# HNUicda/CoIVO

Hardware: AMD Instinct MI355X
Metric: training frame-pairs/sec at 320x256 (higher is better)
Workload: dtype bf16

## Files before the change

### coivo_amd/csrc/wgrad.hip

```cpp
#define COLVO_ACC_CONSTRAINT "+a"
#include "conv_common.h"

namespace colvo {
namespace {

template <typename T, int MT>
constexpr int dy_pitch() {
#ifdef COLVO_WGRAD_OLD_LAYOUT
    return 16 * MT * TT<T>::ES + 16;
#else
    if (TT<T>::ES == 4) return 16 * MT * 4 + 16;
    return MT == 1 ? 32 : MT == 2 ? 96 : 160;
#endif
}

template <typename T, int MT, int NG, bool TAIL, int KS = 1>
__global__ __launch_bounds__(NT * KS) void k_wgrad3x3(const WgradK a) {
    constexpr int G = TT<T>::G, ES = TT<T>::ES;
    constexpr int CK = NG * G;
    constexpr int NCOL = 9 * CK;
    constexpr int NFR = (NCOL + 15) / 16;
    constexpr int FPW = (NFR + 3) / 4;
    constexpr int PIXP = TAIL ? pitch_bytes_s2(NG * 16) : pitch_bytes(NG * 16);
    constexpr int DYP = dy_pitch<T, MT>();
    extern __shared__ __attribute__((aligned(16))) char smem[];
#ifdef COLVO_WTRACE
    long long wt_start = (long long)clock64(), wt_first = 0, wt_store = 0, wt_compute = 0, wt_b1 = 0, wt_b2 = 0, wt_loop_end = 0, wt_flush = 0;
    long long wt_issue = 0, wt_mfma = 0, wt_m0 = 0, wt_m1 = 0;
    long long wt_wall0 = (long long)wall_clock64();
#define WT_STAMP(x) x = (long long)clock64()
#else
#define WT_STAMP(x) do {} while (0)
#endif
    const int tid = threadIdx.x & (NT - 1), lane = tid & 63, wave = tid >> 6;
    const int team = (KS > 1) ? __builtin_amdgcn_readfirstlane(threadIdx.x / NT) : 0;
    const int l15 = lane & 15, kg = lane >> 4;
    const int lid = __builtin_amdgcn_readfirstlane(xcd_remap(blockIdx.x, gridDim.x, a.xcd));
    const int per_split = gridDim.x / a.nsplit;
    const int bsplit = lid / per_split, brem = lid - bsplit * per_split;
    const int bchunk = brem / a.cot, bco = brem - bchunk * a.cot;
    const int co0 = bco * 16 * MT;
    const int chunks0 = a.g.C[0] / CK;
    const int s = (bchunk < chunks0) ? 0 : 1;
    const int c0 = (s == 0 ? bchunk : bchunk - chunks0) * CK;
    const int wc0 = (s == 0 ? 0 : a.g.C[0]) + c0;
    const int S = a.g.stride;
    const int PH = (a.toh - 1) * S + 3, PW = (a.tow - 1) * S + 3;
    const int npix = a.toh * a.tow;
    const int PWL = a.pwl;
    const int stage = (BM * DYP + PH * PWL * PIXP + 15) & ~15;
    char* sDY = smem + team * stage;
    char* sX = sDY + BM * DYP;

    int boff[FPW];
    int ocol[FPW];
#pragma unroll
    for (int fi = 0; fi < FPW; ++fi) {
        const int f = wave + 4 * fi;
        const int ncol_addr = 16 * f + ((ES == 2) ? 4 * (lane & 3) : l15);
        int tap = min(ncol_addr / CK, 8);
        const int c = ncol_addr - (ncol_addr / CK) * CK;
        boff[fi] = ((tap / 3) * PWL + (tap % 3)) * PIXP + c * ES;
        const int ncol = 16 * f + l15;
        ocol[fi] = (f < NFR && ncol < NCOL) ? ((ncol / CK) * a.Ctot + (ncol % CK)) : -1;
    }

    f32x4 acc[MT][FPW];
#pragma unroll
    for (int mi = 0; mi < MT; ++mi)
#pragma unroll
        for (int fi = 0; fi < FPW; ++fi) acc[mi][fi] = f32x4{0.f, 0.f, 0.f, 0.f};
    float dbacc = 0.0f;

    const int t_begin = bsplit * a.tiles_per_split;
    const int t_end = min(a.ntiles, t_begin + a.tiles_per_split);
    const int tiles_per_img = a.tiles_x * a.tiles_y;

    constexpr int DGR = 16 * MT / G;
    constexpr int DIT = (BM * DGR + NT - 1) / NT;
    constexpr int PPF = TAIL ? 9 : 3;
    const int ptotal = PH * PW * NG;
    u32x4 dyv[DIT], pv[PPF];

    struct TileC { int b, ty, tx; };
    auto tile_next = [&](TileC& c) {
        if (++c.tx == a.tiles_x) { c.tx = 0; if (++c.ty == a.tiles_y) { c.ty = 0; ++c.b; } }
    };
    TileC cur;
    {
        const int t = __builtin_amdgcn_readfirstlane(t_begin + team);
        cur.b = t / tiles_per_img;
        const int tr_ = t - cur.b * tiles_per_img;
        cur.ty = tr_ / a.tiles_x; cur.tx = tr_ - cur.ty * a.tiles_x;
    }
    const long long dy_bytes = (long long)a.B * a.Ho * a.Wo * a.Cout * ES;
    const long long x_bytes = (long long)a.B * a.g.Hs[s] * a.g.Ws[s] * a.g.C[s] * ES;
    const __amdgpu_buffer_rsrc_t rdy = __builtin_amdgcn_make_buffer_rsrc((void*)a.dy, 0, (int)(dy_bytes < 0x7fffffffLL ? dy_bytes : 0x7fffffffLL), 0x00020000);
    const __amdgpu_buffer_rsrc_t rx = __builtin_amdgcn_make_buffer_rsrc((void*)a.g.src[s], 0, (int)(x_bytes < 0x7fffffffLL ? x_bytes : 0x7fffffffLL), 0x00020000);
    const int Hs = a.g.Hs[s], Ws = a.g.Ws[s], Cs = a.g.C[s];
    const int sh = (a.g.mode[s] != MODE_DIRECT) ? 1 : 0;

    int dy_off[DIT], dy_yx[DIT], dy_lds[DIT];
#pragma unroll
    for (int it = 0; it < DIT; ++it) {
        const int i = it * NT + tid;
        const int pp_ = i / DGR, gch = i - pp_ * DGR;
        const int oy = mdiv(pp_, a.m_tow), ox = pp_ - oy * a.tow;
        const bool ok = (BM * DGR % NT == 0 || i < BM * DGR) && (pp_ < npix) && (co0 + gch * G < a.Cout);
        dy_off[it] = ok ? ((oy * a.Wo + ox) * a.Cout + co0 + gch * G) * ES : OOB_OFF;
        dy_yx[it] = (oy << 16) | ox;
        dy_lds[it] = pp_ * DYP + gch * 16;
    }
    int p_yx[PPF], p_cg[PPF], p_lds[PPF];
#pragma unroll
    for (int it = 0; it < PPF; ++it) {
        const int i = it * NT + tid;
        const int pix = i / NG;
        p_cg[it] = i - pix * NG;
        const int py = mdiv(pix, a.m_pw), px = pix - py * PW;
        p_yx[it] = (i < ptotal) ? ((py << 16) | px) : (0x7fff << 16);
        p_lds[it] = (py * PWL + px) * PIXP + p_cg[it] * 16;
    }
    auto load_dy = [&](const TileC& c, bool live) {
        const int oy0 = c.ty * a.toh, ox0 = c.tx * a.tow;
        const int base = live ? ((c.b * a.Ho + oy0) * a.Wo + ox0) * a.Cout * ES : 0;
        const int remy = live ? a.Ho - oy0 : 0, remx = a.Wo - ox0;
        if (remy >= a.toh && remx >= a.tow) {
#pragma unroll
            for (int it = 0; it < DIT; ++it) dyv[it] = bld16(rdy, dy_off[it], base);
        } else {
#pragma unroll
            for (int it = 0; it < DIT; ++it) {
                const bool ok = ((dy_yx[it] >> 16) < remy) && ((dy_yx[it] & 0xffff) < remx);
                dyv[it] = bld16(rdy, ok ? dy_off[it] : OOB_OFF, base);
            }
        }
    };
    auto store_dy = [&]() {
#pragma unroll
        for (int it = 0; it < DIT; ++it)
            if (BM * DGR % NT == 0 || it * NT + tid < BM * DGR) st16(sDY + dy_lds[it], dyv[it]);
    };
    auto patch_voff = [&](const TileC& c, int yx, int cg) -> int {
        const int vy = c.ty * a.toh * S - 1 + (yx >> 16), vx = c.tx * a.tow * S - 1 + (yx & 0xffff);
        const bool inb = ((unsigned)vy < (unsigned)a.g.Hi) && ((unsigned)vx < (unsigned)a.g.Wi);
        return inb ? (((vy >> sh) * Ws + (vx >> sh)) * Cs + c0 + cg * G) * ES : OOB_OFF;
    };
    auto load_p = [&](const TileC& c, bool live) {
        const int base = live ? c.b * Hs * Ws * Cs * ES : 0;
        const int dead = live ? 0 : OOB_OFF;
#pragma unroll
        for (int it = 0; it < PPF; ++it) pv[it] = bld16(rx, patch_voff(c, p_yx[it], p_cg[it]) | dead, base);
    };
    auto store_p = [&](const TileC& c, bool live) {
#pragma unroll
        for (int it = 0; it < PPF; ++it) {
            const int i = it * NT + tid;
            if (i < ptotal) st16(sX + p_lds[it], pv[it]);
        }
        const int base = live ? c.b * Hs * Ws * Cs * ES : 0;
        const int dead = live ? 0 : OOB_OFF;
        if constexpr (TAIL)
        for (int g0 = PPF * NT; g0 < ptotal; g0 += 3 * NT) {
            u32x4 tt[3];
            int tl[3];
#pragma unroll
            for (int u = 0; u < 3; ++u) {
                const int i = g0 + u * NT + tid;
                const int pix = i / NG, cg = i - pix * NG;
                const int py = mdiv(pix, a.m_pw), px = pix - py * PW;
                tt[u] = bld16(rx, ((i < ptotal) ? patch_voff(c, (py << 16) | px, cg) : OOB_OFF) | dead, base);
                tl[u] = (py * PWL + px) * PIXP + cg * 16;
            }
#pragma unroll
            for (int u = 0; u < 3; ++u)
                if (g0 + u * NT + tid < ptotal) st16(sX + tl[u], tt[u]);
        }
    };
    constexpr int NPH = NT / (16 * MT);
    const int db_co = tid % (16 * MT), db_ph = tid / (16 * MT);

    if (t_begin < t_end) { const bool live = t_begin + team < t_end; load_dy(cur, live); load_p(cur, live); }
    for (int t = t_begin; t < t_end; t += KS) {
        __syncthreads();
#ifdef COLVO_WTRACE
        WT_STAMP(wt_b1);
        if (t == t_begin) wt_first = wt_b1; else wt_compute += wt_b1 - wt_b2;
#endif
        store_dy();
        store_p(cur, t + team < t_end);
        __syncthreads();
#ifdef COLVO_WTRACE
        WT_STAMP(wt_b2);
        wt_store += wt_b2 - wt_b1;
#endif
#pragma unroll
        for (int q = 0; q < KS; ++q) tile_next(cur);
        if (t + KS < t_end) { const bool live = t + KS + team < t_end; load_dy(cur, live); load_p(cur, live); }

        if (bchunk == 0 && a.db) {
            float s0 = 0.0f, s1 = 0.0f;
#pragma unroll 4
            for (int p = db_ph; p < BM; p += 2 * NPH) {
                if constexpr (ES == 2) {
                    s0 += bf2f(*reinterpret_cast<const uint16_t*>(sDY + p * DYP + db_co * 2));
                    s1 += bf2f(*reinterpret_cast<const uint16_t*>(sDY + (p + NPH) * DYP + db_co * 2));
                } else {
                    s0 += *reinterpret_cast<const float*>(sDY + p * DYP + db_co * 4);
                    s1 += *reinterpret_cast<const float*>(sDY + (p + NPH) * DYP + db_co * 4);
                }
            }
            dbacc += s0 + s1;
        }

#ifdef COLVO_WTRACE
        WT_STAMP(wt_m0);
        wt_issue += wt_m0 - wt_b2;
#endif
        if constexpr (ES == 2) {
            const int q = l15 >> 2, pp = lane & 3;
            auto read_step = [&](int ks, s16x8 (&af)[MT], s16x8 (&bfv)[FPW]) {
                int xo[2], yo[2];
#pragma unroll
                for (int h = 0; h < 2; ++h) {
#ifdef COLVO_WGRAD_OLD_LAYOUT
                    int p = 32 * ks + 8 * kg + q + 4 * h;
#else
                    int p = 32 * ks + 16 * (kg >> 1) + 8 * h + 4 * (kg & 1) + q;
#endif
                    yo[h] = p * DYP;
                    if (p >= npix) p = 0;
                    const int oy = mdiv(p, a.m_tow), ox = p - oy * a.tow;
                    xo[h] = ((oy * S) * PWL + ox * S) * PIXP;
                }
#pragma unroll
                for (int mi = 0; mi < MT; ++mi) {
                    const s16x4 lo = __builtin_amdgcn_ds_read_tr16_b64_v4i16(
                        (__attribute__((address_space(3))) s16x4*)(sDY + yo[0] + (16 * mi + 4 * pp) * 2));
                    const s16x4 hi = __builtin_amdgcn_ds_read_tr16_b64_v4i16(
                        (__attribute__((address_space(3))) s16x4*)(sDY + yo[1] + (16 * mi + 4 * pp) * 2));
                    af[mi] = s16x8{lo[0], lo[1], lo[2], lo[3], hi[0], hi[1], hi[2], hi[3]};
                }
#pragma unroll
                for (int fi = 0; fi < FPW; ++fi) {
                    const s16x4 lo = __builtin_amdgcn_ds_read_tr16_b64_v4i16(
                        (__attribute__((address_space(3))) s16x4*)(sX + xo[0] + boff[fi]));
                    const s16x4 hi = __builtin_amdgcn_ds_read_tr16_b64_v4i16(
                        (__attribute__((address_space(3))) s16x4*)(sX + xo[1] + boff[fi]));
                    bfv[fi] = s16x8{lo[0], lo[1], lo[2], lo[3], hi[0], hi[1], hi[2], hi[3]};
                }
            };
            s16x8 af[MT], bfv[FPW];
#pragma unroll
            for (int ks = 0; ks < 4; ++ks) {
                read_step(ks, af, bfv);
#pragma unroll
                for (int fi = 0; fi < FPW; ++fi)
#pragma unroll
                    for (int mi = 0; mi < MT; ++mi)
                        acc[mi][fi] = __builtin_amdgcn_mfma_f32_16x16x32_bf16(
                            __builtin_bit_cast(bf16x8, af[mi]), __builtin_bit_cast(bf16x8, bfv[fi]), acc[mi][fi], 0, 0, 0);
            }
        } else {
            int p = kg;
            int oy = mdiv(p, a.m_tow), ox = p - oy * a.tow;
            for (int ks = 0; ks < BM / 4; ++ks) {
                const bool live = p < npix;
                const int xo = live ? ((oy * S) * PWL + ox * S) * PIXP : 0;
                float av[MT];
#pragma unroll
                for (int mi = 0; mi < MT; ++mi)
                    av[mi] = *reinterpret_cast<const float*>(sDY + p * DYP + (16 * mi + l15) * 4);
#pragma unroll
                for (int fi = 0; fi < FPW; ++fi) {
                    const float bvv = *reinterpret_cast<const float*>(sX + xo + boff[fi]);
#pragma unroll
                    for (int mi = 0; mi < MT; ++mi)
                        acc[mi][fi] = __builtin_amdgcn_mfma_f32_16x16x4f32(av[mi], bvv, acc[mi][fi], 0, 0, 0);
                }
                p += 4; ox += 4;
                while (ox >= a.tow) { ox -= a.tow; ++oy; }
            }
        }
#ifdef COLVO_WTRACE
        asm volatile("" ::: "memory");
        WT_STAMP(wt_m1);
        wt_mfma += wt_m1 - wt_m0;
#endif
    }

    mfma_result_guard<T>(reinterpret_cast<f32x4 (&)[MT * FPW]>(acc));
#ifdef COLVO_WTRACE
    __syncthreads();
    WT_STAMP(wt_loop_end);
    wt_compute += wt_loop_end - wt_b2;
#endif
    float* sdb = reinterpret_cast<float*>(smem);
    if constexpr (KS > 1) {
        f32x4* sRed = reinterpret_cast<f32x4*>(smem);
        sdb = reinterpret_cast<float*>(smem + MT * FPW * NT * 16);
        for (int g = 1; g < KS; ++g) {
            __syncthreads();
            if (team == g) {
#pragma unroll
                for (int mi = 0; mi < MT; ++mi)
#pragma unroll
                    for (int fi = 0; fi < FPW; ++fi) sRed[(mi * FPW + fi) * NT + tid] = acc[mi][fi];
            }
            __syncthreads();
            if (team == 0) {
#pragma unroll
                for (int mi = 0; mi < MT; ++mi)
#pragma unroll
                    for (int fi = 0; fi < FPW; ++fi) acc[mi][fi] += sRed[(mi * FPW + fi) * NT + tid];
            }
        }
    }
    if (team == 0) {
        auto elem = [&](int mi, int fi, int r, size_t& e) -> bool {
            const int co = co0 + 16 * mi + 4 * kg + r;
            e = (size_t)co * 9 * a.Ctot + wc0 + ocol[fi];
            return ocol[fi] >= 0 && co < a.Cout;
        };
        if (!a.slabs && a.det == 2) {
#pragma unroll
            for (int mi = 0; mi < MT; ++mi)
#pragma unroll
                for (int fi = 0; fi < FPW; ++fi)
#pragma unroll
                    for (int r = 0; r < 4; ++r) { size_t e; if (elem(mi, fi, r, e)) a.dw[e] = acc[mi][fi][r]; }
        } else if (!a.slabs && a.det) {
            float old[MT][FPW][4];
#pragma unroll
            for (int mi = 0; mi < MT; ++mi)
#pragma unroll
                for (int fi = 0; fi < FPW; ++fi)
#pragma unroll
                    for (int r = 0; r < 4; ++r) { size_t e; old[mi][fi][r] = elem(mi, fi, r, e) ? a.dw[e] : 0.0f; }
#pragma unroll
            for (int mi = 0; mi < MT; ++mi)
#pragma unroll
                for (int fi = 0; fi < FPW; ++fi)
#pragma unroll
                    for (int r = 0; r < 4; ++r) { size_t e; if (elem(mi, fi, r, e)) a.dw[e] = old[mi][fi][r] + acc[mi][fi][r]; }
        } else {
#pragma unroll
            for (int mi = 0; mi < MT; ++mi)
#pragma unroll
                for (int fi = 0; fi < FPW; ++fi)
#pragma unroll
                    for (int r = 0; r < 4; ++r) {
                        size_t e;
                        if (!elem(mi, fi, r, e)) continue;
                        if (a.slabs) a.slabs[(size_t)bsplit * a.Cout * 9 * a.Ctot + e] = acc[mi][fi][r];
                        else atomicAdd(a.dw + e, acc[mi][fi][r]);
                    }
        }
    }
    if (bchunk == 0 && a.db) {
        __syncthreads();
        sdb[threadIdx.x] = dbacc;
        __syncthreads();
        if (threadIdx.x < 16 * MT && co0 + tid < a.Cout) {
            float t = 0.0f;
#pragma unroll
            for (int ph = 0; ph < NPH * KS; ++ph) t += sdb[ph * 16 * MT + tid];
            if (a.db_slabs) a.db_slabs[(size_t)bsplit * a.Cout + co0 + tid] = t;
            else if (a.det == 2) a.db[co0 + tid] = t;
            else if (a.det) a.db[co0 + tid] += t;
            else atomicAdd(a.db + co0 + tid, t);
        }
    }
#ifdef COLVO_WTRACE
    if (a.trace) {
        __builtin_amdgcn_s_waitcnt(0);
        __syncthreads();
        WT_STAMP(wt_flush);
        if (threadIdx.x == 0) {
            long long* r = a.trace + (size_t)blockIdx.x * 16;
            r[0] = wt_start; r[1] = wt_first - wt_start; r[2] = wt_store; r[3] = wt_compute; r[4] = wt_flush - wt_loop_end;
            r[5] = wt_flush - wt_start; r[6] = (long long)wall_clock64() - wt_wall0; r[7] = (t_end - t_begin + KS - 1) / KS;
            r[8] = wt_issue; r[9] = wt_mfma;
        }
    }
#endif
}
#undef WT_STAMP

__device__ __forceinline__ void reduce_slabs(const float* __restrict__ slabs, int nsplit, size_t n, float* __restrict__ dst,
                                             size_t first, size_t stride) {
    for (size_t i = first; i < n; i += stride) {
        float t = 0.0f;
        int q = 0;
        for (; q + 8 <= nsplit; q += 8) {
            float v[8];
#pragma unroll
            for (int u = 0; u < 8; ++u) v[u] = slabs[(size_t)(q + u) * n + i];
#pragma unroll
            for (int u = 0; u < 8; ++u) t += v[u];
        }
        for (; q < nsplit; ++q) t += slabs[(size_t)q * n + i];
        dst[i] += t;
    }
}
__global__ __launch_bounds__(NT) void k_wgrad_reduce(const float* __restrict__ slabs, int nsplit, size_t n, float* __restrict__ dst,
                                                     unsigned wblocks, const float* __restrict__ bslabs, size_t nb,
                                                     float* __restrict__ bdst) {
    if (blockIdx.x < wblocks) reduce_slabs(slabs, nsplit, n, dst, (size_t)blockIdx.x * NT + threadIdx.x, (size_t)wblocks * NT);
    else reduce_slabs(bslabs, nsplit, nb, bdst, (size_t)(blockIdx.x - wblocks) * NT + threadIdx.x, (size_t)(gridDim.x - wblocks) * NT);
}

struct ReduceEntry {
    const float* slabs;
    float* dst;
    long long n4;
    int nsplit, sp;
    unsigned blk0;
};
struct ReduceGroup {
    ReduceEntry e[2 * COLVO_WGRAD_GROUP_MAX];
    int n;
};
__global__ __launch_bounds__(NT) void k_wgrad_reduce_group(const ReduceGroup g) {
    __shared__ f32x4 part[NT];
    int ei = 0;
#pragma unroll 1
    for (int i = 1; i < g.n; ++i)
        if (blockIdx.x >= g.e[i].blk0) ei = i;
    const ReduceEntry e = g.e[ei];
    const int qpb = NT / e.sp;
    const int s = threadIdx.x / qpb, ql = threadIdx.x - s * qpb;
    const long long q = (long long)(blockIdx.x - e.blk0) * qpb + ql;
    f32x4 t = f32x4{0.f, 0.f, 0.f, 0.f};
    if (q < e.n4) {
        const f32x4* base = reinterpret_cast<const f32x4*>(e.slabs) + q;
        f32x4 v[8];
        int cnt = 0;
#pragma unroll
        for (int u = 0; u < 8; ++u) {
            const int sp_i = s + u * e.sp;
            if (sp_i < e.nsplit) { v[u] = base[(long long)sp_i * e.n4]; cnt = u + 1; } else v[u] = f32x4{0.f, 0.f, 0.f, 0.f};
        }
#pragma unroll
        for (int u = 0; u < 8; ++u) t += v[u];
        (void)cnt;
        for (int sp_i = s + 8 * e.sp; sp_i < e.nsplit; sp_i += e.sp) t += base[(long long)sp_i * e.n4];
    }
    if (e.sp > 1) {
        part[threadIdx.x] = t;
        __syncthreads();
        if (s == 0) {
            for (int j = 1; j < e.sp; ++j) t += part[j * qpb + ql];
        }
    }
    if (s == 0 && q < e.n4) {
        f32x4* d = reinterpret_cast<f32x4*>(e.dst) + q;
        *d = *d + t;
    }
}

#ifdef COLVO_WTRACE
static long long* g_wtrace = nullptr;
static int g_wtrace_calls = 0;
inline void wtrace_begin(WgradK& k, unsigned nwg, hipStream_t s) {
    k.trace = nullptr;
    if (!getenv("COLVO_WTRACE") || nwg > (1u << 14)) return;
    if (!g_wtrace) (void)hipMalloc(&g_wtrace, (size_t)(1u << 14) * 16 * sizeof(long long));
    (void)hipMemsetAsync(g_wtrace, 0, (size_t)nwg * 16 * sizeof(long long), s);
    k.trace = g_wtrace;
}
inline void wtrace_end(const WgradK& k, unsigned nwg, int MT, int NG, bool tail, int ks, hipStream_t s) {
    if (!k.trace || (++g_wtrace_calls % atoi(getenv("COLVO_WTRACE"))) != 0) return;
    (void)hipStreamSynchronize(s);
    std::vector<long long> h((size_t)nwg * 16);
    (void)hipMemcpy(h.data(), g_wtrace, h.size() * sizeof(long long), hipMemcpyDeviceToHost);
    double m[16] = {0};
    long long t0 = h[0], t1 = 0;
    for (unsigned i = 0; i < nwg; ++i) {
        for (int j = 1; j < 16; ++j) m[j] += (double)h[(size_t)i * 16 + j] / nwg;
        t0 = std::min(t0, h[(size_t)i * 16]); t1 = std::max(t1, h[(size_t)i * 16] + h[(size_t)i * 16 + 5]);
    }
    const double cyc_per_us = m[6] > 0 ? m[5] / (m[6] * 0.01) : 0.0;
    const double nt = std::max(1.0, m[7]);
    fprintf(stderr, "[wtrace] MT=%d NG=%d tail=%d KS=%d S=%d Cout=%d Ctot=%d %dx%d tile %dx%d grid=%u nsplit=%d tiles/wg %.1f | clock %.0f MHz | "
            "mean wg (us): life %.2f = setup+first-load %.2f + store %.2f + compute %.2f + flush %.2f | per tile: store %.3f compute %.3f = "
            "load issue %.3f + MFMA phase %.3f + barrier wait %.3f\n",
            MT, NG, (int)tail, ks, k.g.stride, k.Cout, k.Ctot, k.Ho, k.Wo, k.toh, k.tow, nwg, k.nsplit, m[7], cyc_per_us,
            m[5] / cyc_per_us, m[1] / cyc_per_us, m[2] / cyc_per_us, m[3] / cyc_per_us, m[4] / cyc_per_us, m[2] / cyc_per_us / nt,
            m[3] / cyc_per_us / nt, m[8] / cyc_per_us / nt, m[9] / cyc_per_us / nt, (m[3] - m[8] - m[9]) / cyc_per_us / nt);
}
#endif

inline bool wgrad_prepare(WgradK& k, int nsplit, int* err) {
    *err = 0;
    if (k.plan_out) { *k.plan_out = nsplit; return true; }
    k.slabs = nullptr; k.db_slabs = nullptr;
    k.det = (k.scratch && nsplit == 1 && !k.slabs_only) ? 1 : 0;
    if (k.clean && nsplit == 1 && !k.slabs_only && TUNE(wgrad_store_clean)) k.det = 2;
    if (k.scratch && (nsplit > 1 || k.slabs_only)) {
        const long long wsize = (long long)k.Cout * 9 * k.Ctot;
        const long long need = (long long)nsplit * (wsize + k.Cout) * 4;
        if (need > k.scratch_bytes) {
            set_error("colvo_conv_wgrad_det: scratch of %lld bytes, %lld needed (colvo_conv_wgrad_scratch_bytes)", k.scratch_bytes, need);
            *err = (int)hipErrorInvalidValue;
            return true;
        }
        k.slabs = (float*)const_cast<char*>(k.scratch);
        k.db_slabs = k.slabs + (size_t)nsplit * wsize;
    }
    return false;
}

inline int wgrad_finish(const WgradK& k, int nsplit, hipStream_t s) {
    if (!k.slabs || k.slabs_only) return 0;
    const size_t wsize = (size_t)k.Cout * 9 * k.Ctot;
    const unsigned blocks = (unsigned)std::min<size_t>((wsize + NT - 1) / NT, 2048);
    const unsigned bblocks = k.db ? (unsigned)((k.Cout + NT - 1) / NT) : 0;
    colvo::launch(k_wgrad_reduce, dim3(blocks + bblocks), dim3(NT), 0, s, (const float*)k.slabs, nsplit, wsize, k.dw, blocks,
                       (const float*)k.db_slabs, (size_t)k.Cout, k.db);
    COLVO_CHECK_LAUNCH("k_wgrad_reduce");
    return 0;
}

template <typename T, int MT>
__global__ __launch_bounds__(NT) void k_wgrad_up2(const WgradK a) {
    constexpr int G = TT<T>::G, ES = TT<T>::ES;
    constexpr int NG = 4, CK = NG * G;
    constexpr int NCF = CK / 16;
    constexpr int NACC = 4 * NCF;
    constexpr int PIXP = pitch_bytes(NG * 16);
    constexpr int DYP = dy_pitch<T, MT>();
    extern __shared__ __attribute__((aligned(16))) char smem[];
    const int tid = threadIdx.x, lane = tid & 63;
    const int cls = __builtin_amdgcn_readfirstlane(tid >> 6);
    const int cpy = cls >> 1, cpx = cls & 1;
    const int l15 = lane & 15, kg = lane >> 4;
    const int lid = __builtin_amdgcn_readfirstlane(xcd_remap(blockIdx.x, gridDim.x, a.xcd));
    const int per_split = gridDim.x / a.nsplit;
    const int bsplit = lid / per_split, brem = lid - bsplit * per_split;
    const int bchunk = brem / a.cot, bco = brem - bchunk * a.cot;
    const int co0 = bco * 16 * MT;
    const int c0 = bchunk * CK;
    const int PH = a.toh + 2, PW = a.tow + 2;
    const int PWL = a.pwl;
    const int npix = a.toh * a.tow;
    char* sDY = smem;
    char* sX = smem + 4 * BM * DYP;

    f32x4 acc[MT][NACC];
#pragma unroll
    for (int mi = 0; mi < MT; ++mi)
#pragma unroll
        for (int q = 0; q < NACC; ++q) acc[mi][q] = f32x4{0.f, 0.f, 0.f, 0.f};
    float dbacc = 0.0f;

    const int t_begin = bsplit * a.tiles_per_split;
    const int t_end = min(a.ntiles, t_begin + a.tiles_per_split);
    const int tiles_per_img = a.tiles_x * a.tiles_y;
    constexpr int DGR = 16 * MT / G;
    constexpr int DIT = 4 * BM * DGR / NT;
    constexpr int PPF = 3;
    const int ptotal = PH * PW * NG;
    u32x4 dyv[DIT], pv[PPF];
    struct TileC { int b, ty, tx; };
    auto tile_next = [&](TileC& c) {
        if (++c.tx == a.tiles_x) { c.tx = 0; if (++c.ty == a.tiles_y) { c.ty = 0; ++c.b; } }
    };
    TileC cur;
    {
        const int t = __builtin_amdgcn_readfirstlane(t_begin);
        cur.b = t / tiles_per_img;
        const int tr_ = t - cur.b * tiles_per_img;
        cur.ty = tr_ / a.tiles_x; cur.tx = tr_ - cur.ty * a.tiles_x;
    }
    const int Hs = a.g.Hs[0], Ws = a.g.Ws[0], Cs = a.g.C[0];
    const long long dy_bytes = (long long)a.B * a.Ho * a.Wo * a.Cout * ES;
    const long long x_bytes = (long long)a.B * Hs * Ws * Cs * ES;
    const __amdgpu_buffer_rsrc_t rdy = __builtin_amdgcn_make_buffer_rsrc((void*)a.dy, 0, (int)(dy_bytes < 0x7fffffffLL ? dy_bytes : 0x7fffffffLL), 0x00020000);
    const __amdgpu_buffer_rsrc_t rx = __builtin_amdgcn_make_buffer_rsrc((void*)a.g.src[0], 0, (int)(x_bytes < 0x7fffffffLL ? x_bytes : 0x7fffffffLL), 0x00020000);

    int dy_off[DIT], dy_yx[DIT], dy_lds[DIT];
#pragma unroll
    for (int it = 0; it < DIT; ++it) {
        const int i = it * NT + tid;
        const int c4 = i / (BM * DGR), rem = i - c4 * (BM * DGR);
        const int pos = rem / DGR, gch = rem - pos * DGR;
        const int oy = mdiv(pos, a.m_tow), ox = pos - oy * a.tow;
        const bool ok = (pos < npix) && (co0 + gch * G < a.Cout);
        dy_off[it] = ok ? (((2 * oy + (c4 >> 1)) * a.Wo + 2 * ox + (c4 & 1)) * a.Cout + co0 + gch * G) * ES : OOB_OFF;
        dy_yx[it] = (oy << 16) | ox;
        dy_lds[it] = (c4 * BM + pos) * DYP + gch * 16;
    }
    int p_yx[PPF], p_cg[PPF], p_lds[PPF];
#pragma unroll
    for (int it = 0; it < PPF; ++it) {
        const int i = it * NT + tid;
        const int pix = i / NG;
        p_cg[it] = i - pix * NG;
        const int py = mdiv(pix, a.m_pw), px = pix - py * PW;
        p_yx[it] = (i < ptotal) ? ((py << 16) | px) : (0x7fff << 16);
        p_lds[it] = (py * PWL + px) * PIXP + p_cg[it] * 16;
    }
    auto load_tile = [&](const TileC& c) {
        const int oy0 = c.ty * a.toh, ox0 = c.tx * a.tow;
        {
            const int base = ((c.b * a.Ho + 2 * oy0) * a.Wo + 2 * ox0) * a.Cout * ES;
            const int remy = Hs - oy0, remx = Ws - ox0;
            if (remy >= a.toh && remx >= a.tow) {
#pragma unroll
                for (int it = 0; it < DIT; ++it) dyv[it] = bld16(rdy, dy_off[it], base);
            } else {
#pragma unroll
                for (int it = 0; it < DIT; ++it) {
                    const bool ok = ((dy_yx[it] >> 16) < remy) && ((dy_yx[it] & 0xffff) < remx);
                    dyv[it] = bld16(rdy, ok ? dy_off[it] : OOB_OFF, base);
                }
            }
        }
        const int base = c.b * Hs * Ws * Cs * ES;
#pragma unroll
        for (int it = 0; it < PPF; ++it) {
            const int vy = oy0 - 1 + (p_yx[it] >> 16), vx = ox0 - 1 + (p_yx[it] & 0xffff);
            const bool inb = ((unsigned)vy < (unsigned)Hs) && ((unsigned)vx < (unsigned)Ws);
            pv[it] = bld16(rx, inb ? ((vy * Ws + vx) * Cs + c0 + p_cg[it] * G) * ES : OOB_OFF, base);
        }
    };
    constexpr int NPH = NT / (16 * MT);
    const int db_co = tid % (16 * MT), db_ph = tid / (16 * MT);

    if (t_begin < t_end) load_tile(cur);
    for (int t = t_begin; t < t_end; ++t) {
        __syncthreads();
#pragma unroll
        for (int it = 0; it < DIT; ++it) st16(sDY + dy_lds[it], dyv[it]);
#pragma unroll
        for (int it = 0; it < PPF; ++it)
            if (it * NT + tid < ptotal) st16(sX + p_lds[it], pv[it]);
        __syncthreads();
        tile_next(cur);
        if (t + 1 < t_end) load_tile(cur);

        if (bchunk == 0 && a.db) {
            float s0 = 0.0f;
#pragma unroll 4
            for (int p = db_ph; p < 4 * BM; p += NPH) {
                if constexpr (ES == 2) s0 += bf2f(*reinterpret_cast<const uint16_t*>(sDY + p * DYP + db_co * 2));
                else s0 += *reinterpret_cast<const float*>(sDY + p * DYP + db_co * 4);
            }
            dbacc += s0;
        }

        const char* sDYc = sDY + cls * BM * DYP;
        if constexpr (ES == 2) {
            const int q = l15 >> 2, pp = lane & 3;
            auto read_step = [&](int ks, s16x8 (&af)[MT], s16x8 (&bfv)[NACC]) {
                int xo[2], yo[2];
#pragma unroll
                for (int h = 0; h < 2; ++h) {
                    int p = 32 * ks + 16 * (kg >> 1) + 8 * h + 4 * (kg & 1) + q;
                    yo[h] = p * DYP;
                    if (p >= npix) p = 0;
                    const int oy = mdiv(p, a.m_tow), ox = p - oy * a.tow;
                    xo[h] = ((oy + cpy) * PWL + ox + cpx) * PIXP;
                }
#pragma unroll
                for (int mi = 0; mi < MT; ++mi) {
                    const s16x4 lo = __builtin_amdgcn_ds_read_tr16_b64_v4i16(
                        (__attribute__((address_space(3))) s16x4*)(sDYc + yo[0] + (16 * mi + 4 * pp) * 2));
                    const s16x4 hi = __builtin_amdgcn_ds_read_tr16_b64_v4i16(
                        (__attribute__((address_space(3))) s16x4*)(sDYc + yo[1] + (16 * mi + 4 * pp) * 2));
                    af[mi] = s16x8{lo[0], lo[1], lo[2], lo[3], hi[0], hi[1], hi[2], hi[3]};
                }
#pragma unroll
                for (int tp = 0; tp < 4; ++tp)
#pragma unroll
                    for (int f = 0; f < NCF; ++f) {
                        const int bo = ((tp >> 1) * PWL + (tp & 1)) * PIXP + (16 * f + 4 * pp) * 2;
                        const s16x4 lo = __builtin_amdgcn_ds_read_tr16_b64_v4i16((__attribute__((address_space(3))) s16x4*)(sX + xo[0] + bo));
                        const s16x4 hi = __builtin_amdgcn_ds_read_tr16_b64_v4i16((__attribute__((address_space(3))) s16x4*)(sX + xo[1] + bo));
                        bfv[tp * NCF + f] = s16x8{lo[0], lo[1], lo[2], lo[3], hi[0], hi[1], hi[2], hi[3]};
                    }
            };
            s16x8 af[2][MT], bfv[2][NACC];
            read_step(0, af[0], bfv[0]);
#pragma unroll
            for (int ks = 0; ks < 4; ++ks) {
                if (ks + 1 < 4) read_step(ks + 1, af[(ks + 1) & 1], bfv[(ks + 1) & 1]);
                __builtin_amdgcn_sched_barrier(0);
#pragma unroll
                for (int qq = 0; qq < NACC; ++qq)
#pragma unroll
                    for (int mi = 0; mi < MT; ++mi)
                        acc[mi][qq] = __builtin_amdgcn_mfma_f32_16x16x32_bf16(
                            __builtin_bit_cast(bf16x8, af[ks & 1][mi]), __builtin_bit_cast(bf16x8, bfv[ks & 1][qq]), acc[mi][qq], 0, 0, 0);
                __builtin_amdgcn_sched_barrier(0);
            }
        } else {
            int p = kg;
            int oy = mdiv(p, a.m_tow), ox = p - oy * a.tow;
            for (int ks = 0; ks < BM / 4; ++ks) {
                const bool live = p < npix;
                const int xo = live ? ((oy + cpy) * PWL + ox + cpx) * PIXP : 0;
                float av[MT];
#pragma unroll
                for (int mi = 0; mi < MT; ++mi) av[mi] = *reinterpret_cast<const float*>(sDYc + p * DYP + (16 * mi + l15) * 4);
#pragma unroll
                for (int tp = 0; tp < 4; ++tp)
#pragma unroll
                    for (int f = 0; f < NCF; ++f) {
                        const float bvv = *reinterpret_cast<const float*>(sX + xo + ((tp >> 1) * PWL + (tp & 1)) * PIXP + (16 * f + l15) * 4);
#pragma unroll
                        for (int mi = 0; mi < MT; ++mi)
                            acc[mi][tp * NCF + f] = __builtin_amdgcn_mfma_f32_16x16x4f32(av[mi], bvv, acc[mi][tp * NCF + f], 0, 0, 0);
                    }
                p += 4; ox += 4;
                while (ox >= a.tow) { ox -= a.tow; ++oy; }
            }
        }
    }

    mfma_result_guard<T>(reinterpret_cast<f32x4 (&)[MT * NACC]>(acc));
    __syncthreads();
    f32x4* sEx = reinterpret_cast<f32x4*>(smem);
    {
        f32x4* mine = sEx + (size_t)cls * 4 * MT * NCF * 64;
#pragma unroll
        for (int tp = 0; tp < 4; ++tp)
#pragma unroll
            for (int mi = 0; mi < MT; ++mi)
#pragma unroll
                for (int f = 0; f < NCF; ++f) mine[((tp * MT + mi) * NCF + f) * 64 + lane] = acc[mi][tp * NCF + f];
    }
    __syncthreads();
    constexpr int NBLK = 9 * MT * NCF;
    for (int blk = cls; blk < NBLK; blk += 4) {
        const int tap = blk / (MT * NCF), rem = blk - tap * (MT * NCF);
        const int mi = rem / NCF, f = rem - mi * NCF;
        const int ky = tap / 3, kx = tap - 3 * ky;
        f32x4 sum = f32x4{0.f, 0.f, 0.f, 0.f};
#pragma unroll
        for (int c4 = 0; c4 < 4; ++c4) {
            const int py = c4 >> 1, px = c4 & 1;
            const int r = py == 0 ? (ky >= 1) : (ky >= 2), c = px == 0 ? (kx >= 1) : (kx >= 2);
            sum += sEx[(((size_t)c4 * 4 + (r * 2 + c)) * MT + mi) * NCF * 64 + f * 64 + lane];
        }
        const size_t e0 = (size_t)(co0 + 16 * mi + 4 * kg) * 9 * a.Ctot + (size_t)tap * a.Ctot + c0 + 16 * f + l15;
        const size_t erow = (size_t)9 * a.Ctot;
        const int nrow = min(4, a.Cout - (co0 + 16 * mi + 4 * kg));
        if (a.slabs) {
#pragma unroll
            for (int rr = 0; rr < 4; ++rr)
                if (rr < nrow) a.slabs[(size_t)bsplit * a.Cout * 9 * a.Ctot + e0 + rr * erow] = sum[rr];
        } else if (a.det == 2) {
#pragma unroll
            for (int rr = 0; rr < 4; ++rr)
                if (rr < nrow) a.dw[e0 + rr * erow] = sum[rr];
        } else if (a.det) {
            float old[4];
#pragma unroll
            for (int rr = 0; rr < 4; ++rr) old[rr] = rr < nrow ? a.dw[e0 + rr * erow] : 0.0f;
#pragma unroll
            for (int rr = 0; rr < 4; ++rr)
                if (rr < nrow) a.dw[e0 + rr * erow] = old[rr] + sum[rr];
        } else {
#pragma unroll
            for (int rr = 0; rr < 4; ++rr)
                if (rr < nrow) atomicAdd(a.dw + e0 + rr * erow, sum[rr]);
        }
    }
    if (bchunk == 0 && a.db) {
        __syncthreads();
        float* sdb = reinterpret_cast<float*>(smem);
        sdb[tid] = dbacc;
        __syncthreads();
        if (tid < 16 * MT && co0 + tid < a.Cout) {
            float t = 0.0f;
#pragma unroll
            for (int ph = 0; ph < NPH; ++ph) t += sdb[ph * 16 * MT + tid];
            if (a.db_slabs) a.db_slabs[(size_t)bsplit * a.Cout + co0 + tid] = t;
            else if (a.det == 2) a.db[co0 + tid] = t;
            else if (a.det) a.db[co0 + tid] += t;
            else atomicAdd(a.db + co0 + tid, t);
        }
    }
}

struct GridFloor { int wgs; bool halved; };
static inline GridFloor wgrad_grid_floor(int base, int ntiles, int per_split) {
    const int short_walk = (int)TUNE(wgrad_short_walk);
    const int nsplit_at_base = std::max(1, (base + per_split - 1) / per_split);
    const bool halved = short_walk > 0 && ntiles / nsplit_at_base < short_walk;
    return {halved ? std::max(1, base / 2) : base, halved};
}

static inline int wgrad_atomic_splits(const WgradK& k, int per_split, bool& halved) {
    const double wbytes = (double)k.Cout * 9.0 * k.Ctot * 4.0;
    const GridFloor lo_wgs = wgrad_grid_floor((int)TUNE(wgrad_wg_lo), k.ntiles, per_split);
    halved = lo_wgs.halved;
    int nsplit = (int)(TUNE_F(wgrad_atomic_mb) * 1e6 / wbytes);
    const int lo = (lo_wgs.wgs + per_split - 1) / per_split, hi = ((int)TUNE(wgrad_wg_hi) + per_split - 1) / per_split;
    if (nsplit > hi) nsplit = hi;
    if (nsplit < lo) nsplit = lo;
    return nsplit;
}

enum { WGRAD_RT, WGRAD_UP2, WGRAD_TEAMS, WGRAD_TAIL };
struct WgradPlan {
    int form;
    int mt, ng;
    bool tail;
    size_t lds;
    int nsplit;
    unsigned nwg;
    bool halved;
    WgradRtPlan rt;
};

inline void set_wgrad_tile(WgradK& k, const Tile& t, int Ho, int Wo, int pw) {
    k.toh = t.toh; k.tow = t.tow;
    k.tiles_x = (Wo + t.tow - 1) / t.tow; k.tiles_y = (Ho + t.toh - 1) / t.toh;
    k.ntiles = k.B * k.tiles_x * k.tiles_y;
    k.m_tow = mdiv_magic(t.tow); k.m_pw = mdiv_magic(pw);
    k.pwl = wgrad_row_pitch(pw, t.tow);
}

inline void set_wgrad_grid(WgradK& k, WgradPlan& p, int nsplit, int cot, int chunks) {
    if (nsplit > k.ntiles) nsplit = k.ntiles;
    if (nsplit < 1) nsplit = 1;
    k.tiles_per_split = (k.ntiles + nsplit - 1) / nsplit;
    p.nsplit = k.nsplit = (k.ntiles + k.tiles_per_split - 1) / k.tiles_per_split;
    k.cot = cot; k.xcd = (int)TUNE(xcd_remap);
    p.nwg = (unsigned)(p.nsplit * cot * chunks);
}

template <typename T>
int dy_pitch_of(int mt) { return mt == 4 ? dy_pitch<T, 4>() : mt == 2 ? dy_pitch<T, 2>() : dy_pitch<T, 1>(); }

template <typename T>
int wgrad_plan(const ColvoConvDesc* d, WgradK& k, WgradPlan& p) {
    constexpr int G = TT<T>::G;
    const bool up2_form = TUNE(wgrad_up2) && d->up0 && d->C1 == 0 && d->stride == 1 && d->C0 % (4 * G) == 0 && d->Cout >= 16;
    if ((!up2_form || TUNE(wgrad_rt_over_up2)) && wgrad_rt_plan(d, p.rt)) {
        p.form = WGRAD_RT;
        p.nsplit = p.rt.nsplit;
        return 0;
    }
    if (up2_form) {
        const int Hs = d->Hi / 2, Ws = d->Wi / 2;
        const Tile t = pick_tile(Hs, Ws, 1, false);
        if ((t.toh + 2) * (t.tow + 2) * 4 <= 3 * NT) {
            constexpr int CK = 4 * G;
            set_wgrad_tile(k, t, Hs, Ws, t.tow + 2);
            p.form = WGRAD_UP2;
            p.mt = d->Cout >= 32 ? 2 : 1;
            p.ng = 4;
            p.lds = std::max((size_t)4 * BM * dy_pitch_of<T>(p.mt) + (size_t)(k.toh + 2) * k.pwl * pitch_bytes(64),
                             (size_t)16 * p.mt * (CK / 16) * 64 * 16) + 64;
            COLVO_CHECK_ARG(p.lds <= 160 * 1024, "wgrad (up-sampled source): tile needs %zu bytes of LDS", p.lds);
            const int chunks = k.g.C[0] / CK, cot = (k.Cout + 16 * p.mt - 1) / (16 * p.mt);
            set_wgrad_grid(k, p, wgrad_atomic_splits(k, chunks * cot, p.halved), cot, chunks);
            return 0;
        }
    }
    const Tile t = pick_tile(d->Ho, d->Wo, d->stride, false);
    set_wgrad_tile(k, t, d->Ho, d->Wo, (t.tow - 1) * d->stride + 3);
    const int ng_max = (int)TUNE(wgrad_ng_max);
    int ng = ng_max;
    for (int i = 0; i < 2; ++i)
        if (k.g.C[i] > 0) while (ng > 1 && (k.g.C[i] % (ng * G)) != 0) ng >>= 1;
    for (int i = 0; i < 2; ++i)
        COLVO_CHECK_ARG(k.g.C[i] % (ng * G) == 0, "wgrad: channel count %d is not a multiple of %d", k.g.C[i], G);
    const int mt_max = (int)TUNE(wgrad_mt_max);
    const int one_chunk_rule = (int)TUNE(wgrad_one_chunk_rule);
    const bool one_chunk = one_chunk_rule && (k.g.C[0] + k.g.C[1]) == ng * G;
    const long walk = (long)k.ntiles * ((k.g.C[0] + k.g.C[1]) / (ng * G)) * ((k.Cout + 63) / 64) / 256;
    if (k.Cout >= 64 && (mt_max >= 4 || walk >= TUNE(wgrad_mt4_min_walk))) p.mt = 4;
    else if (k.Cout >= 32 && mt_max >= 2 && !one_chunk) p.mt = 2;
    else p.mt = 1;
    p.ng = (ng == 4 || ng == 2) ? ng : 1;
    const int S = d->stride, CK = p.ng * G;
    const int PH = (k.toh - 1) * S + 3, PW = k.pwl;
    p.tail = (long)PH * ((k.tow - 1) * S + 3) * p.ng > 3 * NT;
    const int PIXP = p.tail ? pitch_bytes_s2(p.ng * 16) : pitch_bytes(p.ng * 16), DYP = dy_pitch_of<T>(p.mt);
    const int chunks = (k.g.C[0] + k.g.C[1]) / CK;
    const int cot = (k.Cout + 16 * p.mt - 1) / (16 * p.mt);
    const size_t stage = ((size_t)BM * DYP + (size_t)PH * PW * PIXP + 15) & ~(size_t)15;
    const int teams = (int)TUNE(wgrad_teams);
    const int max_slabs = (int)TUNE(wgrad_team_max_slabs);
    if (!p.tail && p.mt == 1 && teams >= 4 && chunks * cot <= max_slabs && stage * 4 + 64 <= 160 * 1024) {
        constexpr int KS = 4;
        const int FPW = ((9 * CK + 15) / 16 + 3) / 4;
        p.form = WGRAD_TEAMS;
        p.lds = std::max(stage * KS, (size_t)p.mt * FPW * NT * 16 + (size_t)NT * KS * 4) + 64;
        COLVO_CHECK_ARG(p.lds <= 160 * 1024, "wgrad: %d teams need %zu bytes of LDS", KS, p.lds);
        const GridFloor target = wgrad_grid_floor((int)TUNE(wgrad_team_wgs), k.ntiles, chunks * cot);
        p.halved = target.halved;
        set_wgrad_grid(k, p, std::max(1, target.wgs / (chunks * cot)), cot, chunks);
        return 0;
    }
    p.form = WGRAD_TAIL;
    p.lds = (size_t)BM * DYP + (size_t)PH * PW * PIXP + 64;
    COLVO_CHECK_ARG(p.lds <= 160 * 1024, "wgrad: tile needs %zu bytes of LDS", p.lds);
    set_wgrad_grid(k, p, wgrad_atomic_splits(k, chunks * cot, p.halved), cot, chunks);
    return 0;
}

template <typename T, int MT, int NG, bool TAIL, int KS = 1>
int launch_wgrad3x3(WgradK& k, const WgradPlan& p, hipStream_t s) {
    if (int e = allow_dynamic_lds<k_wgrad3x3<T, MT, NG, TAIL, KS>>(p.lds, 160 * 1024, "wgrad")) return e;
#ifdef COLVO_WTRACE
    wtrace_begin(k, p.nwg, s);
#endif
    colvo::launch((k_wgrad3x3<T, MT, NG, TAIL, KS>), dim3(p.nwg), dim3(NT * KS), p.lds, s, k);
    COLVO_CHECK_LAUNCH(KS > 1 ? "k_wgrad3x3 (teams)" : "k_wgrad3x3");
#ifdef COLVO_WTRACE
    wtrace_end(k, p.nwg, MT, NG, TAIL, KS, s);
#endif
    return 0;
}

template <typename T, int MT>
int launch_wgrad_up2(const WgradK& k, const WgradPlan& p, hipStream_t s) {
    if (int e = allow_dynamic_lds<k_wgrad_up2<T, MT>>(p.lds, 160 * 1024, "wgrad")) return e;
    colvo::launch((k_wgrad_up2<T, MT>), dim3(p.nwg), dim3(NT), p.lds, s, k);
    COLVO_CHECK_LAUNCH("k_wgrad_up2");
    return 0;
}

template <typename T, int MT>
int launch_wgrad_ng(WgradK& k, const WgradPlan& p, hipStream_t s) {
    switch (p.ng) {
        case 4: return p.tail ? launch_wgrad3x3<T, MT, 4, true>(k, p, s) : launch_wgrad3x3<T, MT, 4, false>(k, p, s);
        case 2: return p.tail ? launch_wgrad3x3<T, MT, 2, true>(k, p, s) : launch_wgrad3x3<T, MT, 2, false>(k, p, s);
        default: return p.tail ? launch_wgrad3x3<T, MT, 1, true>(k, p, s) : launch_wgrad3x3<T, MT, 1, false>(k, p, s);
    }
}

template <typename T>
int launch_wgrad_t(WgradK& k, const WgradPlan& p, hipStream_t s) {
    if (p.form == WGRAD_UP2) return p.mt == 2 ? launch_wgrad_up2<T, 2>(k, p, s) : launch_wgrad_up2<T, 1>(k, p, s);
    if (p.form == WGRAD_TEAMS) {
        switch (p.ng) {
            case 4: return launch_wgrad3x3<T, 1, 4, false, 4>(k, p, s);
            case 2: return launch_wgrad3x3<T, 1, 2, false, 4>(k, p, s);
            default: return launch_wgrad3x3<T, 1, 1, false, 4>(k, p, s);
        }
    }
    switch (p.mt) {
        case 4: return launch_wgrad_ng<T, 4>(k, p, s);
        case 2: return launch_wgrad_ng<T, 2>(k, p, s);
        default: return launch_wgrad_ng<T, 1>(k, p, s);
    }
}

}
}

using namespace colvo;

static int wgrad_impl(const ColvoConvDesc* d, const void* x0, const void* x1, const void* dy, float* dw, float* db,
                      void* scratch, size_t scratch_bytes, int* plan_out, colvo_stream_t stream, int slabs_only = 0, int clean = 0);

extern "C" int colvo_conv_wgrad(const ColvoConvDesc* d, const void* x0, const void* x1, const void* dy, float* dw,
                                float* db, colvo_stream_t stream) {
    return wgrad_impl(d, x0, x1, dy, dw, db, nullptr, 0, nullptr, stream);
}

extern "C" int colvo_conv_wgrad_clean(const ColvoConvDesc* d, const void* x0, const void* x1, const void* dy, float* dw,
                                      float* db, int arena_is_zero, colvo_stream_t stream) {
    return wgrad_impl(d, x0, x1, dy, dw, db, nullptr, 0, nullptr, stream, 0, arena_is_zero ? 1 : 0);
}

extern "C" int colvo_conv_wgrad_det(const ColvoConvDesc* d, const void* x0, const void* x1, const void* dy, float* dw,
                                    float* db, void* scratch, size_t scratch_bytes, colvo_stream_t stream) {
    COLVO_CHECK_ARG(scratch, "colvo_conv_wgrad_det: null scratch");
    return wgrad_impl(d, x0, x1, dy, dw, db, scratch, scratch_bytes, nullptr, stream);
}

extern "C" int colvo_conv_wgrad_slabs(const ColvoConvDesc* d, const void* x0, const void* x1, const void* dy, void* scratch,
                                      size_t scratch_bytes, colvo_stream_t stream) {
    COLVO_CHECK_ARG(scratch, "colvo_conv_wgrad_slabs: null scratch");
    static const float dummy = 0.0f;
    return wgrad_impl(d, x0, x1, dy, const_cast<float*>(&dummy), const_cast<float*>(&dummy), scratch, scratch_bytes, nullptr, stream, 1);
}

extern "C" int colvo_conv_wgrad_splits(const ColvoConvDesc* d) {
    if (!d || check_desc(d, "colvo_conv_wgrad_splits")) return 0;
    int nsplit = 0;
    static const char dummy = 0;
    if (wgrad_impl(d, &dummy, d->C1 ? &dummy : nullptr, &dummy, (float*)&dummy, nullptr, nullptr, 0, &nsplit, nullptr)) return 0;
    return nsplit;
}

extern "C" int colvo_wgrad_reduce_group(const ColvoWgradSlabs* sets, int n, colvo_stream_t stream) {
    COLVO_CHECK_ARG(sets && n >= 1 && n <= COLVO_WGRAD_GROUP_MAX, "colvo_wgrad_reduce_group: 1..%d sets", COLVO_WGRAD_GROUP_MAX);
    ReduceGroup g{};
    unsigned blk = 0;
    auto add = [&](const float* slabs, float* dst, long long n, int nsplit) {
        ReduceEntry& e = g.e[g.n++];
        e.slabs = slabs; e.dst = dst; e.n4 = n / 4; e.nsplit = nsplit;
        int sp = 1;
        while (sp < 64 && sp * 8 < nsplit) sp *= 2;
        if (e.n4 < NT / sp) { while (sp < 64 && (long long)(NT / (sp * 2)) >= e.n4 && sp * 2 <= nsplit) sp *= 2; }
        e.sp = sp;
        e.blk0 = blk;
        blk += (unsigned)((e.n4 + NT / sp - 1) / (NT / sp));
    };
    for (int i = 0; i < n; ++i) {
        const ColvoWgradSlabs& w = sets[i];
        COLVO_CHECK_ARG(w.scratch && w.dw && w.nsplit >= 1 && w.Cout >= 8 && w.Cout % 4 == 0 && w.Ctot >= 8 && w.Ctot % 4 == 0,
                        "colvo_wgrad_reduce_group: bad set %d", i);
        const long long wsize = (long long)w.Cout * 9 * w.Ctot;
        const float* slabs = (const float*)w.scratch;
        COLVO_CHECK_ARG(((uintptr_t)slabs % 16) == 0 && ((uintptr_t)w.dw % 16) == 0 && (!w.db || ((uintptr_t)w.db % 16) == 0),
                        "colvo_wgrad_reduce_group: set %d is not 16-byte aligned", i);
        add(slabs, w.dw, wsize, w.nsplit);
        if (w.db) add(slabs + (size_t)w.nsplit * wsize, w.db, w.Cout, w.nsplit);
    }
    colvo::launch(k_wgrad_reduce_group, dim3(blk), dim3(NT), 0, (hipStream_t)stream, g);
    COLVO_CHECK_LAUNCH("k_wgrad_reduce_group");
    return 0;
}

extern "C" size_t colvo_conv_wgrad_scratch_bytes(const ColvoConvDesc* d) {
    if (!d || check_desc(d, "colvo_conv_wgrad_scratch_bytes")) return 0;
    int nsplit = 0;
    static const char dummy = 0;
    if (wgrad_impl(d, &dummy, d->C1 ? &dummy : nullptr, &dummy, (float*)&dummy, nullptr, nullptr, 0, &nsplit, nullptr)) return 0;
    return (size_t)nsplit * ((size_t)d->Cout * 9 * (d->C0 + d->C1) + d->Cout) * 4;
}

static int wgrad_impl(const ColvoConvDesc* d, const void* x0, const void* x1, const void* dy, float* dw, float* db,
                      void* scratch, size_t scratch_bytes, int* plan_out, colvo_stream_t stream, int slabs_only, int clean) {
    if (int e = check_desc(d, "colvo_conv_wgrad")) return e;
    COLVO_CHECK_ARG(x0 && dy && dw && (d->C1 == 0 || x1), "colvo_conv_wgrad: null pointer argument");
    {
        const long long es = d->dtype == COLVO_F32 ? 4 : 2;
        const long long cmax = d->C0 > d->C1 ? d->C0 : d->C1;
        const long long per_img = std::max((long long)d->Ho * d->Wo * d->Cout, (long long)d->Hi * d->Wi * cmax) * es;
        COLVO_CHECK_ARG(per_img < 0x40000000LL, "colvo_conv_wgrad: a single image of %lld bytes is not supported", per_img);
        const int bmax = (int)std::max(1LL, (0x40000000LL - 1) / per_img);
        if (d->B > bmax) {
            if (!plan_out) form_hit(FORM_WGRAD_SLICED);
            COLVO_CHECK_ARG(!slabs_only, "colvo_conv_wgrad_slabs: batch %d would be sliced (tensors >= 1 GiB); use colvo_conv_wgrad_det", d->B);
            const long long e0 = (long long)(d->up0 ? (d->Hi / 2) * (d->Wi / 2) : d->Hi * d->Wi) * d->C0 * es;
            const long long e1 = (long long)(d->up1 ? (d->Hi / 2) * (d->Wi / 2) : d->Hi * d->Wi) * d->C1 * es;
            const long long ey = (long long)d->Ho * d->Wo * d->Cout * es;
            for (int b0 = 0; b0 < d->B; b0 += bmax) {
                ColvoConvDesc sub = *d;
                sub.B = std::min(bmax, d->B - b0);
                int plan = 0;
                if (int e = wgrad_impl(&sub, (const char*)x0 + b0 * e0, x1 ? (const char*)x1 + b0 * e1 : nullptr,
                                       (const char*)dy + b0 * ey, dw, db, scratch, scratch_bytes, plan_out ? &plan : nullptr, stream, 0,
                                       b0 == 0 ? clean : 0))
                    return e;
                if (plan_out) *plan_out = std::max(*plan_out, plan);
            }
            return 0;
        }
    }
    WgradK k{};
    fill_gather(d, x0, d->C1 ? x1 : nullptr, k.g);
    k.Ho = d->Ho; k.Wo = d->Wo; k.B = d->B;
    k.dy = (const char*)dy; k.Cout = d->Cout; k.dw = dw; k.Ctot = d->C0 + d->C1; k.db = db;
    k.scratch = (const char*)scratch; k.scratch_bytes = scratch ? (long long)scratch_bytes : 0; k.plan_out = plan_out;
    k.slabs_only = slabs_only;
    k.clean = clean;
    WgradPlan p{};
    if (int e = d->dtype == COLVO_F32 ? wgrad_plan<float>(d, k, p) : wgrad_plan<bf16_t>(d, k, p)) return e;
    { int err; if (wgrad_prepare(k, p.nsplit, &err)) return err; }
    const hipStream_t s = (hipStream_t)stream;
    if (p.form == WGRAD_RT) {
        form_hit(FORM_WGRAD_RT);
        if (int e = wgrad_rt_launch(p.rt, d, x0, d->C1 ? x1 : nullptr, dy, dw, db, k.slabs, k.db_slabs, k.det, s)) return e;
    } else {
        form_hit(p.form == WGRAD_UP2 ? FORM_WGRAD_UP2 : p.form == WGRAD_TEAMS ? FORM_WGRAD_TEAMS : FORM_WGRAD_TAIL);
        if (p.form == WGRAD_TAIL && p.mt == 4) form_hit(FORM_WGRAD_MT4);
        form_hit(p.halved ? FORM_WGRAD_HALVED_GRID : FORM_WGRAD_FULL_GRID);
        if (k.det == 2) form_hit(FORM_WGRAD_STORE_CLEAN);
        if (int e = d->dtype == COLVO_F32 ? launch_wgrad_t<float>(k, p, s) : launch_wgrad_t<bf16_t>(k, p, s)) return e;
    }
    return wgrad_finish(k, p.nsplit, s);
}
```

Measured before the change: 5684.

## Split wgrad slab reduction across thread groups with LDS combine for large split counts

Moves the split-K weight-gradient slab reduction into a new header, where each block can assign several thread groups to different slabs of the same output elements and combine their partial sums through LDS. It also unrolls the loads 16 deep with clamped indices, so each thread has more independent loads in flight. The goal is more memory-level parallelism when nsplit is large and the output is small, at the cost of extra barriers and redundant clamped loads when nsplit is not a multiple of the unroll.

```diff
diff --git a/coivo_amd/csrc/wgrad.hip b/coivo_amd/csrc/wgrad.hip
--- a/coivo_amd/csrc/wgrad.hip
+++ b/coivo_amd/csrc/wgrad.hip
@@ -1,5 +1,6 @@
 #define COLVO_ACC_CONSTRAINT "+a"
 #include "conv_common.h"
+#include "wgrad_reduce.h"
 
 namespace colvo {
 namespace {
@@ -387,28 +388,6 @@
 }
 #undef WT_STAMP
 
-__device__ __forceinline__ void reduce_slabs(const float* __restrict__ slabs, int nsplit, size_t n, float* __restrict__ dst,
-                                             size_t first, size_t stride) {
-    for (size_t i = first; i < n; i += stride) {
-        float t = 0.0f;
-        int q = 0;
-        for (; q + 8 <= nsplit; q += 8) {
-            float v[8];
-#pragma unroll
-            for (int u = 0; u < 8; ++u) v[u] = slabs[(size_t)(q + u) * n + i];
-#pragma unroll
-            for (int u = 0; u < 8; ++u) t += v[u];
-        }
-        for (; q < nsplit; ++q) t += slabs[(size_t)q * n + i];
-        dst[i] += t;
-    }
-}
-__global__ __launch_bounds__(NT) void k_wgrad_reduce(const float* __restrict__ slabs, int nsplit, size_t n, float* __restrict__ dst,
-                                                     unsigned wblocks, const float* __restrict__ bslabs, size_t nb,
-                                                     float* __restrict__ bdst) {
-    if (blockIdx.x < wblocks) reduce_slabs(slabs, nsplit, n, dst, (size_t)blockIdx.x * NT + threadIdx.x, (size_t)wblocks * NT);
-    else reduce_slabs(bslabs, nsplit, nb, bdst, (size_t)(blockIdx.x - wblocks) * NT + threadIdx.x, (size_t)(gridDim.x - wblocks) * NT);
-}
 
 struct ReduceEntry {
     const float* slabs;
@@ -514,10 +493,14 @@
 inline int wgrad_finish(const WgradK& k, int nsplit, hipStream_t s) {
     if (!k.slabs || k.slabs_only) return 0;
     const size_t wsize = (size_t)k.Cout * 9 * k.Ctot;
-    const unsigned blocks = (unsigned)std::min<size_t>((wsize + NT - 1) / NT, 2048);
-    const unsigned bblocks = k.db ? (unsigned)((k.Cout + NT - 1) / NT) : 0;
-    colvo::launch(k_wgrad_reduce, dim3(blocks + bblocks), dim3(NT), 0, s, (const float*)k.slabs, nsplit, wsize, k.dw, blocks,
-                       (const float*)k.db_slabs, (size_t)k.Cout, k.db);
+    using namespace colvo_reduce;
+    const ReduceForm f = reduce_form(nsplit);
+    const int sg = f.sg;
+    const unsigned blocks = reduce_blocks(wsize, sg);
+    const unsigned bblocks = k.db ? reduce_blocks((size_t)k.Cout, sg) : 0;
+    auto kern = reduce_kernel(f);
+    colvo::launch(kern, dim3(blocks + bblocks), dim3(colvo_reduce::RED_NT), 0, s, (const float*)k.slabs, nsplit, wsize, k.dw, blocks,
+                  (const float*)k.db_slabs, (size_t)k.Cout, k.db);
     COLVO_CHECK_LAUNCH("k_wgrad_reduce");
     return 0;
 }
diff --git a/coivo_amd/csrc/wgrad_reduce.h b/coivo_amd/csrc/wgrad_reduce.h
--- /dev/null
+++ b/coivo_amd/csrc/wgrad_reduce.h
@@ -0,0 +1,68 @@
+#pragma once
+#include <hip/hip_runtime.h>
+
+namespace colvo_reduce {
+
+constexpr int RED_NT = 256;
+
+struct ReduceForm { int sg, u; };
+inline ReduceForm reduce_form(int nsplit) { return {nsplit <= 16 ? 1 : nsplit <= 64 ? 4 : 16, 16}; }
+
+template <int SG, int RED_U>
+__device__ __forceinline__ void reduce_slabs(const float* __restrict__ slabs, int nsplit, size_t n, float* __restrict__ dst,
+                                             size_t first_tile, size_t tile_stride, float* __restrict__ lds) {
+    constexpr int E = RED_NT / SG;
+    const int e = (int)threadIdx.x % E, g = (int)threadIdx.x / E;
+    const size_t ntiles = (n + E - 1) / E;
+    for (size_t tile = first_tile; tile < ntiles; tile += tile_stride) {
+        const size_t i = tile * E + e, ic = i < n ? i : n - 1;
+        const float d0 = dst[ic];
+        float t = 0.0f;
+        for (int q0 = 0; q0 < nsplit; q0 += SG * RED_U) {
+            float v[RED_U];
+#pragma unroll
+            for (int u = 0; u < RED_U; ++u) {
+                const int q = min(q0 + u * SG + g, nsplit - 1);
+                v[u] = slabs[(size_t)q * n + ic];
+            }
+            if constexpr (SG == 1) {
+#pragma unroll
+                for (int u = 0; u < RED_U; ++u)
+                    if (q0 + u < nsplit) t += v[u];
+            } else {
+                if (q0) __syncthreads();
+#pragma unroll
+                for (int u = 0; u < RED_U; ++u) lds[(u * SG + g) * E + e] = v[u];
+                __syncthreads();
+                if (g == 0) {
+                    const int m = min(SG * RED_U, nsplit - q0);
+#pragma unroll 16
+                    for (int j = 0; j < m; ++j) t += lds[j * E + e];
+                }
+            }
+        }
+        if (g == 0 && i < n) dst[i] = d0 + t;
+        if constexpr (SG > 1) __syncthreads();
+    }
+}
+
+template <int SG, int RED_U>
+__global__ __launch_bounds__(RED_NT) void k_wgrad_reduce(const float* __restrict__ slabs, int nsplit, size_t n, float* __restrict__ dst,
+                                                         unsigned wblocks, const float* __restrict__ bslabs, size_t nb,
+                                                         float* __restrict__ bdst) {
+    __shared__ float lds[SG > 1 ? RED_NT * RED_U : 1];
+    if (blockIdx.x < wblocks) reduce_slabs<SG, RED_U>(slabs, nsplit, n, dst, blockIdx.x, wblocks, lds);
+    else reduce_slabs<SG, RED_U>(bslabs, nsplit, nb, bdst, blockIdx.x - wblocks, gridDim.x - wblocks, lds);
+}
+
+typedef void (*ReduceKernel)(const float*, int, size_t, float*, unsigned, const float*, size_t, float*);
+inline ReduceKernel reduce_kernel(ReduceForm f) {
+    return f.sg == 1 ? k_wgrad_reduce<1, 16> : f.sg == 4 ? k_wgrad_reduce<4, 16> : k_wgrad_reduce<16, 16>;
+}
+
+inline unsigned reduce_blocks(size_t n, int sg) {
+    const size_t e = RED_NT / sg;
+    return (unsigned)((n + e - 1) / e < 2048 ? (n + e - 1) / e : 2048);
+}
+
+}
```

After: 5729, median of 6. Within noise of the previous version (+0.8%).
